# pinellolab/GRAFIMO

Hardware: AMD Instinct MI355X
Metric: scored haplotype k-mers/sec (higher is better)
Workload: dtype int32

## Files before the change

grafimo_amd/csrc/gfm_score_kernels.hpp:

```cpp
#pragma once

#include "gfm_common.hpp"

namespace {

constexpr int kWave = 64;
constexpr int kThreads = 1024;
constexpr int kWavesPerWG = kThreads / kWave;
constexpr unsigned kPoison = 0xFFFFu;
constexpr int kMaxLdsBytes = 160 * 1024;
constexpr int kWGsPerCU = 1;
constexpr int kReserveCUs = 4;
constexpr int kHitQueue = 64;

constexpr int kWorkspaces = GFM_WORKSPACE_RING;
constexpr int kCtlSlots = 2 * GFM_WORKSPACE_RING;
constexpr int kCtlAhead = GFM_WORKSPACE_RING;
struct HitCtl {
    unsigned long long mid[kCtlSlots];
    unsigned long long snap[kCtlSlots];
};
constexpr int kResidPerWG = kWavesPerWG * kHitQueue;

__device__ inline void hitq_push(long long *hitq, int &qn, bool hit, long long entry, int lane,
                                 const unsigned long long *hit_count, unsigned long long *mid,
                                 long long *hit_rows, long long hit_cap)
{
    const unsigned long long mask = __builtin_amdgcn_ballot_w64(hit);
    if (!mask) return;
    const int nh = __popcll(mask);
    if (qn + nh > kHitQueue) {
        unsigned long long base = 0;
        if (lane == 0) base = (hit_count ? *hit_count : 0ull) + atomicAdd(mid, (unsigned long long)qn);
        base = __shfl(base, 0);
        for (int i = lane; i < qn; i += kWave)
            if ((long long)(base + i) < hit_cap) hit_rows[base + i] = hitq[i];
        qn = 0;
    }
    if (hit) hitq[qn + __popcll(mask & ((1ull << lane) - 1ull))] = entry;
    qn += nh;
}

template <int WAVES>
__device__ inline void hitq_finish(const long long *hitq, int qn, int *wq_n ,
                                   int wave, int lane, int tid, long long *resid, int *resid_n)
{
    if (lane == 0) wq_n[wave] = qn;
    __syncthreads();
    int base = 0, tot = 0;
#pragma unroll
    for (int w = 0; w < WAVES; ++w) {
        if (w < wave) base += wq_n[w];
        tot += wq_n[w];
    }
    long long *slab = resid + (size_t)blockIdx.x * kResidPerWG;
    for (int i = lane; i < qn; i += kWave) slab[base + i] = hitq[i];
    if (tid == 0) resid_n[blockIdx.x] = tot;
}

constexpr int kSpillCopies = 16;

struct MotifArgs {
    const uint16_t *tab;
    int lo, nb, min_val;
    int use_hist;
    int spill_lo;
    int spill_n;
    unsigned *spill;
    int cutoff;
    int slot;
    int *scores;
    unsigned *partials;
    long long *hit_rows;
    long long hit_cap;
    const unsigned long long *hit_count;
    HitCtl *ctl;
    long long *resid;
    int *resid_n;
};
template <int MM> struct ScoreArgs {
    MotifArgs m[MM];
    int store_through;
};

typedef __attribute__((address_space(3))) const unsigned lds_cu32;
typedef __attribute__((address_space(3))) const uint16_t lds_cu16;
typedef __attribute__((address_space(3))) const unsigned long long lds_cu64;
__device__ inline unsigned lds_offset(const void *p)
{
    return (unsigned)(size_t)(__attribute__((address_space(3))) const char *)p;
}

constexpr int kSlabsPerGroup = 16;
constexpr int kPostJobs = 3;
struct PostJob {
    const unsigned *partials;
    unsigned long long *hist64;
    unsigned *spill;
    const long long *resid;
    const int *resid_n;
    HitCtl *ctl;
    long long *hit_rows;
    unsigned long long *hit_count;
    long long hit_cap;
    int nslabs, nb, lo, min_val, bin_blocks, hist_blocks, spill_lo, spill_n, spill_blocks, hit_slabs, par, total;
};
struct PostJobs { PostJob j[kPostJobs]; };

__device__ inline void
post_body(const unsigned *__restrict__ partials, int nslabs, int nb, int lo, int min_val,
          unsigned long long *__restrict__ hist64, int bin_blocks, int hist_blocks,
          unsigned *__restrict__ spill, int spill_lo, int spill_n, int spill_blocks,
          const long long *__restrict__ resid, const int *__restrict__ resid_n, int hit_slabs,
          HitCtl *__restrict__ ctl, int par, long long *__restrict__ hit_rows, long long hit_cap,
          unsigned long long *__restrict__ hit_count)
{
    const int tid = threadIdx.x;
    if (blockIdx.x == 0 && tid == 0 && hit_slabs == 0 && ctl) ctl->mid[(par + kCtlAhead) % kCtlSlots] = 0ull;
    if ((int)blockIdx.x < hist_blocks) {
        const int bx = blockIdx.x % bin_blocks, by = blockIdx.x / bin_blocks;
        const int b = bx * 256 + tid;
        if (b > nb) return;
        const int g0 = by * kSlabsPerGroup;
        const int g1 = min(g0 + kSlabsPerGroup, nslabs);
        unsigned long long s = 0;
        const size_t stride = (size_t)(nb + 1);
#pragma unroll 8
        for (int g = g0; g < g1; ++g) s += __builtin_nontemporal_load(&partials[g * stride + b]);
        if (s) atomicAdd(&hist64[b == nb ? min_val : lo + b], s);
        return;
    }
    if ((int)blockIdx.x < hist_blocks + spill_blocks) {
        const int b = ((int)blockIdx.x - hist_blocks) * 256 + tid;
        if (b < spill_n) {
            unsigned long long v = 0;
#pragma unroll
            for (int c = 0; c < kSpillCopies; ++c) {
                const unsigned x = spill[(size_t)c * (size_t)spill_n + b];
                if (x) {
                    v += x;
                    spill[(size_t)c * (size_t)spill_n + b] = 0u;
                }
            }
            if (v) atomicAdd(&hist64[spill_lo + b], v);
        }
        return;
    }
    __shared__ int part[256];
    __shared__ int part_all[256];
    const int g = blockIdx.x - hist_blocks - spill_blocks;
    int s = 0, sa = 0;
    for (int k = tid; k < hit_slabs; k += 256) {
        const int v = resid_n[k];
        sa += v;
        if (k < g) s += v;
    }
    part[tid] = s;
    part_all[tid] = sa;
    __syncthreads();
    for (int d = 128; d > 0; d >>= 1) {
        if (tid < d) { part[tid] += part[tid + d]; part_all[tid] += part_all[tid + d]; }
        __syncthreads();
    }
    const unsigned long long start = ctl->snap[par] + ctl->mid[par];
    const unsigned long long base = start + (unsigned long long)part[0];
    const int cnt = resid_n[g];
    const long long *slab = resid + (size_t)g * kResidPerWG;
    for (int i = tid; i < cnt; i += 256)
        if ((long long)(base + i) < hit_cap) __builtin_nontemporal_store(__builtin_nontemporal_load(&slab[i]), &hit_rows[base + i]);
    if (g == 0 && tid == 0) {
        *hit_count = start + (unsigned long long)part_all[0];
        ctl->mid[(par + kCtlAhead) % kCtlSlots] = 0ull;
    }
}

__global__ void __launch_bounds__(256) post_kernel(const PostJobs jobs)
{
    const PostJob &q = jobs.j[blockIdx.y];
    if ((int)blockIdx.x >= q.total) return;
    post_body(q.partials, q.nslabs, q.nb, q.lo, q.min_val, q.hist64, q.bin_blocks, q.hist_blocks, q.spill, q.spill_lo,
              q.spill_n, q.spill_blocks, q.resid, q.resid_n, q.hit_slabs, q.ctl, q.par, q.hit_rows, q.hit_cap,
              q.hit_count);
}

constexpr int kSelThreads = 256;
__global__ void __launch_bounds__(kSelThreads)
select_hits_kernel(const int *__restrict__ scores, long long n, const int *__restrict__ cutoff_ptr,
                   long long row_base, long long *__restrict__ hit_rows, long long hit_cap,
                   const unsigned long long *__restrict__ hit_count, HitCtl *__restrict__ ctl,
                   int par, long long *__restrict__ resid, int *__restrict__ resid_n,
                   const unsigned long long *__restrict__ gate_count, long long gate_cap)
{
    __shared__ long long hq[kSelThreads / kWave][kHitQueue];
    __shared__ int wq_n[kSelThreads / kWave];
    const int cutoff = *cutoff_ptr;
    const int tid = threadIdx.x, lane = tid & 63, wave = tid >> 6;
    long long *hitq = hq[wave];
    int qn = 0;
    if (gate_count) {
        if ((long long)*gate_count <= gate_cap) {
            if (tid == 0) {
                resid_n[blockIdx.x] = 0;
                if (blockIdx.x == 0) ctl->snap[par] = hit_count ? *hit_count : 0ull;
            }
            return;
        }
        hit_count = nullptr;
    }
    if (blockIdx.x == 0 && tid == 0) ctl->snap[par] = hit_count ? *hit_count : 0ull;
    const long long nthreads = (long long)gridDim.x * blockDim.x;
    const long long n4 = (n + 3) >> 2;
    const long long iters = (n4 + nthreads - 1) / nthreads;
    const long long t0 = (long long)blockIdx.x * blockDim.x + tid;
    for (long long it = 0; it < iters; ++it) {
        const long long i = t0 + it * nthreads;
        int sc[4] = {INT32_MIN, INT32_MIN, INT32_MIN, INT32_MIN};
        if (i * 4 + 4 <= n) {
            const int4 v = reinterpret_cast<const int4 *>(scores)[i];
            sc[0] = v.x; sc[1] = v.y; sc[2] = v.z; sc[3] = v.w;
        } else {
            for (int j = 0; j < 4; ++j)
                if (i * 4 + j < n) sc[j] = scores[i * 4 + j];
        }
#pragma unroll
        for (int j = 0; j < 4; ++j)
            hitq_push(hitq, qn, sc[j] >= cutoff,
                      ((row_base + i * 4 + j) << GFM_HIT_SCORE_BITS) | (long long)sc[j], lane,
                      hit_count, &ctl->mid[par], hit_rows, hit_cap);
    }
    hitq_finish<kSelThreads / kWave>(hitq, qn, wq_n, wave, lane, tid, resid, resid_n);
}

constexpr int kFilterPerThread = 16;
constexpr int kFilterPerBlock = kSelThreads * kFilterPerThread;
__global__ void __launch_bounds__(kSelThreads)
filter_hits_kernel(const long long *__restrict__ cand, const unsigned long long *__restrict__ cand_count,
                   long long cand_cap, const int *__restrict__ cutoff_ptr, long long *__restrict__ hit_rows,
                   long long hit_cap, unsigned long long *__restrict__ hit_count)
{
    __shared__ int wave_tot[kSelThreads / kWave];
    __shared__ unsigned long long block_base;
    const int cutoff = *cutoff_ptr;
    const int tid = threadIdx.x, lane = tid & 63, wave = tid >> 6;
    const unsigned long long have = *cand_count;
    if ((long long)have > cand_cap) {
        if (blockIdx.x == 0 && tid == 0) *hit_count = have;
        return;
    }
    const long long n = (long long)have;
    const long long first = (long long)blockIdx.x * kFilterPerBlock;
    if (first >= n) return;
    long long e[kFilterPerThread];
    int mine = 0;
#pragma unroll
    for (int j = 0; j < kFilterPerThread; ++j) {
        const long long i = first + (long long)j * kSelThreads + tid;
        e[j] = i < n ? cand[i] : -1ll;
        const bool keep = i < n && (int)(e[j] & ((1ll << GFM_HIT_SCORE_BITS) - 1)) >= cutoff;
        if (!keep) e[j] = -1ll;
        mine += keep ? 1 : 0;
    }
    int incl = mine;
#pragma unroll
    for (int d = 1; d < kWave; d <<= 1) {
        const int v = __shfl_up(incl, d);
        if (lane >= d) incl += v;
    }
    if (lane == kWave - 1) wave_tot[wave] = incl;
    __syncthreads();
    int before = 0, total = 0;
#pragma unroll
    for (int w = 0; w < kSelThreads / kWave; ++w) {
        if (w < wave) before += wave_tot[w];
        total += wave_tot[w];
    }
    if (tid == 0) block_base = total ? atomicAdd(hit_count, (unsigned long long)total) : 0ull;
    __syncthreads();
    unsigned long long at = block_base + (unsigned long long)(before + incl - mine);
#pragma unroll
    for (int j = 0; j < kFilterPerThread; ++j)
        if (e[j] >= 0) {
            if ((long long)at < hit_cap) hit_rows[at] = e[j];
            ++at;
        }
}

}
```

grafimo_amd/csrc/gfm_score_quad.hpp:

```cpp
#pragma once

#include "gfm_score_kernels.hpp"
#include "gfm_quad_launch.hpp"

namespace {

typedef unsigned u32x2_t __attribute__((ext_vector_type(2)));
typedef unsigned u32x4_t __attribute__((ext_vector_type(4)));
typedef __attribute__((address_space(3))) const u32x2_t lds_cu32x2;
typedef __attribute__((address_space(3))) const u32x4_t lds_cu32x4;
typedef int i32x4 __attribute__((ext_vector_type(4)));

template <int W, int MM, bool STORE = true>
__global__ void __launch_bounds__(kThreads)
score_quad_kernel(const uint8_t *__restrict__ kmers, long long n, long long row_base, const ScoreArgs<MM> a)
{
    extern __shared__ __attribute__((aligned(16))) unsigned char smem[];
    constexpr int NDW = (W + 3) / 4;
    constexpr int kTabBytes = quad_tab_bytes(W, MM);
    constexpr int CB = kQuadRows * W;
    constexpr int kLoads = (CB + 1023) / 1024;
    constexpr int GP = quad_pitch(W);
    constexpr int PAD = quad_pad(W);
    constexpr int SSTRIDE = quad_strip_stride(W, MM);

    if (lds_offset(smem) != 0u) __builtin_trap();
    const int tid = threadIdx.x;
    const int lane = tid & (kWave - 1);
    const int wave = __builtin_amdgcn_readfirstlane(tid >> 6);
    const int n_waves = (int)(blockDim.x >> 6);
    const int wg_threads = (int)blockDim.x;
    unsigned char *tab = smem;
    unsigned char *stage_base = smem + kTabBytes;
    unsigned *hist[MM];
    {
        unsigned *h = reinterpret_cast<unsigned *>(stage_base + n_waves * SSTRIDE);
#pragma unroll
        for (int m = 0; m < MM; ++m) {
            hist[m] = h;
            if (a.m[m].use_hist) h += a.m[m].nb + 1;
        }
    }

    unsigned char *stage = stage_base + wave * SSTRIDE;
    const unsigned stage_off = (unsigned)(kTabBytes + wave * SSTRIDE);
    const long long nfull = n / kQuadRows;
    const long long cstride = (long long)gridDim.x * n_waves;
    bool vec_store = true;
    const bool through = a.store_through == 1;
    constexpr bool no_store = !STORE;
#pragma unroll
    for (int m = 0; m < MM; ++m) vec_store = vec_store && (reinterpret_cast<uintptr_t>(a.m[m].scores) & 15u) == 0;

    uint4 pre[kQuadDepth][kLoads];
    auto fetch = [&](uint4 (&dst)[kLoads], long long c) {
        const uint8_t *src = kmers + c * (long long)CB + lane * 16;
#pragma unroll
        for (int i = 0; i < kLoads; ++i) {
            if (i * 1024 + 1024 <= CB || i * 1024 + lane * 16 < CB) {
                typedef unsigned u32x4 __attribute__((ext_vector_type(4)));
                const u32x4 t = __builtin_nontemporal_load(reinterpret_cast<const u32x4 *>(src + i * 1024));
                dst[i] = make_uint4(t.x, t.y, t.z, t.w);
            }
        }
    };

    long long *hitq[MM];
    int qn[MM];
    bool select[MM];
#pragma unroll
    for (int m = 0; m < MM; ++m) {
        hitq[m] = reinterpret_cast<long long *>(stage + quad_stage_bytes(W)) + m * kHitQueue;
        qn[m] = 0;
        select[m] = a.m[m].cutoff != GFM_NO_SELECT;
        if (select[m] && blockIdx.x == 0 && tid == 0)
            a.m[m].ctl->snap[a.m[m].slot] = a.m[m].hit_count ? *a.m[m].hit_count : 0ull;
    }

    int p_score[MM][4];
    long long p_crow = -1;
    auto book = [&]() {
        const int k0 = 4 * lane;
#pragma unroll
        for (int m = 0; m < MM; ++m) {
            const MotifArgs &ma = a.m[m];
            if (ma.use_hist) {
#pragma unroll
                for (int j = 0; j < 4; ++j) {
                    const unsigned off = (unsigned)(p_score[m][j] - ma.lo);
                    if (off < (unsigned)ma.nb)
                        atomicAdd(&hist[m][off], 1u);
                    else if (p_score[m][j] == ma.min_val)
                        atomicAdd(&hist[m][ma.nb], 1u);
                    else
                        atomicAdd(&ma.spill[(size_t)(blockIdx.x & (kSpillCopies - 1)) * (size_t)ma.spill_n + (size_t)(p_score[m][j] - ma.spill_lo)], 1u);
                }
            }
            if (select[m]) {
                const int best = max(max(p_score[m][0], p_score[m][1]), max(p_score[m][2], p_score[m][3]));
                if (__builtin_amdgcn_ballot_w64(best >= ma.cutoff)) {
#pragma unroll
                    for (int j = 0; j < 4; ++j)
                        hitq_push(hitq[m], qn[m], p_score[m][j] >= ma.cutoff,
                                  ((row_base + p_crow + k0 + j) << GFM_HIT_SCORE_BITS) | (long long)p_score[m][j], lane,
                                  ma.hit_count, &ma.ctl->mid[ma.slot], ma.hit_rows, ma.hit_cap);
                }
            }
        }
    };

    long long c = (long long)blockIdx.x * n_waves + wave;
#pragma unroll
    for (int d = 0; d < kQuadDepth; ++d)
        if (c + d * cstride < nfull) fetch(pre[d], c + d * cstride);
    if constexpr (MM == 1) {
        for (int i = tid; i < kTabBytes / 2; i += wg_threads) reinterpret_cast<uint16_t *>(tab)[i] = a.m[0].tab[i];
    } else {
        for (int i = tid; i < kTabBytes / 8; i += wg_threads) {
            unsigned long long v = 0;
            if (a.m[0].tab[i] == kPoison) {
                v = 1ull << 57;
            } else {
#pragma unroll
                for (int m = 0; m < MM; ++m) v |= (unsigned long long)a.m[m].tab[i] << (19 * m);
            }
            reinterpret_cast<unsigned long long *>(tab)[i] = v;
        }
    }
#pragma unroll
    for (int m = 0; m < MM; ++m)
        if (a.m[m].use_hist)
            for (int i = tid; i <= a.m[m].nb; i += wg_threads) hist[m][i] = 0u;
    __syncthreads();

    while (c < nfull) {
#pragma unroll
        for (int d = 0; d < kQuadDepth; ++d) {
            if (c >= nfull) break;
            const long long crow = c * kQuadRows;
            if (p_crow >= 0) book();
#pragma unroll
            for (int i = 0; i < kLoads; ++i) {
                const int off = i * 1024 + lane * 16;
                if (i * 1024 + 1024 <= CB || off < CB) {
                    const int dst = PAD ? off + PAD * (off / (4 * W)) : off;
                    *reinterpret_cast<uint4 *>(stage + dst) = pre[d][i];
                }
            }
            if (c + kQuadDepth * cstride < nfull) fetch(pre[d], c + kQuadDepth * cstride);
            __builtin_amdgcn_fence(__ATOMIC_RELEASE, "wavefront");
            __builtin_amdgcn_wave_barrier();

            unsigned w[W + 1];
            {
                const unsigned base = stage_off + (unsigned)(lane * GP);
                if constexpr (W % 2 == 1) {
#pragma unroll
                    for (int t = 0; t < W; ++t) w[t] = ((lds_cu32 *)(uintptr_t)base)[t];
                } else if constexpr (W % 4 == 2) {
#pragma unroll
                    for (int t = 0; t < W / 2; ++t) {
                        const u32x2_t v = ((lds_cu32x2 *)(uintptr_t)base)[t];
                        w[2 * t] = v.x;
                        w[2 * t + 1] = v.y;
                    }
                } else {
#pragma unroll
                    for (int t = 0; t < W / 4; ++t) {
                        const u32x4_t v = ((lds_cu32x4 *)(uintptr_t)base)[t];
                        w[4 * t] = v.x;
                        w[4 * t + 1] = v.y;
                        w[4 * t + 2] = v.z;
                        w[4 * t + 3] = v.w;
                    }
                }
                w[W] = 0u;
            }
            int score[MM][4];
#pragma unroll
            for (int j = 0; j < 4; ++j) {
                const int r = (j * W) & 3;
                bool any_n;
                int acc[MM];
                if constexpr (MM == 1) {
                    int s1 = 0;
#pragma unroll
                    for (int t = 0; t < NDW; ++t) {
                        const int q = (j * W + 4 * t) >> 2;
                        const unsigned x = r ? __builtin_amdgcn_alignbit(w[q + 1], w[q], (unsigned)(8 * r)) : w[q];
                        unsigned y;
                        asm("v_bfi_b32 %0, %1, %2, %3" : "=v"(y) : "s"(0x000E000Eu), "v"(x), "v"(x >> 5));
                        const unsigned e0 = y & 0x7Eu;
                        const unsigned e1 = (y >> 16) & 0x7Eu;
                        s1 += *(lds_cu16 *)(uintptr_t)(e0 + (unsigned)((2 * t) * 128));
                        s1 += *(lds_cu16 *)(uintptr_t)(e1 + (unsigned)((2 * t + 1) * 128));
                    }
                    any_n = (unsigned)s1 >= kPoison;
                    acc[0] = s1;
                } else {
                    unsigned long long s64 = 0;
#pragma unroll
                    for (int t = 0; t < NDW; ++t) {
                        const int q = (j * W + 4 * t) >> 2;
                        const unsigned x = r ? __builtin_amdgcn_alignbit(w[q + 1], w[q], (unsigned)(8 * r)) : w[q];
                        unsigned y;
                        asm("v_bfi_b32 %0, %1, %2, %3" : "=v"(y) : "s"(0x000E000Eu), "v"(x), "v"(x >> 5));
                        const unsigned e0 = (y & 0x7Eu) << 2;
                        const unsigned e1 = ((y >> 16) & 0x7Eu) << 2;
                        s64 += *(lds_cu64 *)(uintptr_t)(e0 + (unsigned)((2 * t) * 512));
                        s64 += *(lds_cu64 *)(uintptr_t)(e1 + (unsigned)((2 * t + 1) * 512));
                    }
                    any_n = (s64 >> 57) != 0;
#pragma unroll
                    for (int m = 0; m < MM; ++m) acc[m] = (int)((s64 >> (19 * m)) & 0x7FFFFull);
                }
#pragma unroll
                for (int m = 0; m < MM; ++m) score[m][j] = any_n ? a.m[m].min_val : acc[m];
            }
            const int k0 = 4 * lane;
#pragma unroll
            for (int m = 0; m < MM; ++m) {
                const __amdgpu_buffer_rsrc_t rs =
                    __builtin_amdgcn_make_buffer_rsrc(a.m[m].scores + crow, 0, kQuadRows * 4, 0x00020000);
                if (no_store) {
                } else if (vec_store) {
                    const u32x4_t out = {(unsigned)score[m][0], (unsigned)score[m][1], (unsigned)score[m][2],
                                         (unsigned)score[m][3]};
                    if (through)
                        __builtin_amdgcn_raw_buffer_store_b128(out, rs, k0 * 4, 0, kStoreThrough);
                    else
                        __builtin_amdgcn_raw_buffer_store_b128(out, rs, k0 * 4, 0, kStoreStream);
                } else {
#pragma unroll
                    for (int j = 0; j < 4; ++j) {
                        if (through)
                            __builtin_amdgcn_raw_buffer_store_b32((unsigned)score[m][j], rs, (k0 + j) * 4, 0, kStoreThrough);
                        else
                            __builtin_amdgcn_raw_buffer_store_b32((unsigned)score[m][j], rs, (k0 + j) * 4, 0, kStoreStream);
                    }
                }
#pragma unroll
                for (int j = 0; j < 4; ++j) p_score[m][j] = score[m][j];
            }
            p_crow = crow;
            __builtin_amdgcn_fence(__ATOMIC_ACQUIRE, "wavefront");
            __builtin_amdgcn_wave_barrier();
            c += cstride;
        }
    }
    if (p_crow >= 0) book();
    if (blockIdx.x == gridDim.x - 1 && wave == n_waves - 1 && nfull * kQuadRows < n) {
        const long long first = nfull * kQuadRows;
        const int count = (int)(n - first);
#pragma unroll 1
        for (int r0 = 0; r0 < count; r0 += kWave) {
            const int k = r0 + lane;
            const bool live = k < count;
            const uint8_t *row = kmers + (first + (live ? k : 0)) * (long long)W;
            unsigned long long s64 = 0;
            bool bad = false;
#pragma unroll 1
            for (int p = 0; p < 2 * NDW; ++p) {
                const unsigned b0 = 2 * p < W ? row[2 * p] : (unsigned)'A';
                const unsigned b1 = 2 * p + 1 < W ? row[2 * p + 1] : (unsigned)'A';
                const unsigned e = p * 64 + ((b0 >> 1) & 7u) + 8u * ((b1 >> 1) & 7u);
                if constexpr (MM == 1) {
                    const unsigned v = reinterpret_cast<const uint16_t *>(tab)[e];
                    bad = bad || v == kPoison;
                    s64 += v;
                } else {
                    s64 += reinterpret_cast<const unsigned long long *>(tab)[e];
                }
            }
            if constexpr (MM > 1) bad = (s64 >> 57) != 0;
#pragma unroll
            for (int m = 0; m < MM; ++m) {
                const MotifArgs &ma = a.m[m];
                const int sc = bad ? ma.min_val : (int)((MM == 1 ? s64 : (s64 >> (19 * m))) & 0x7FFFFull);
                if (live) {
                    if (!no_store) ma.scores[first + k] = sc;
                    if (ma.use_hist) {
                        const unsigned off = (unsigned)(sc - ma.lo);
                        if (off < (unsigned)ma.nb)
                            atomicAdd(&hist[m][off], 1u);
                        else if (sc == ma.min_val)
                            atomicAdd(&hist[m][ma.nb], 1u);
                        else
                            atomicAdd(&ma.spill[(size_t)(blockIdx.x & (kSpillCopies - 1)) * (size_t)ma.spill_n + (size_t)(sc - ma.spill_lo)], 1u);
                    }
                }
                if (select[m])
                    hitq_push(hitq[m], qn[m], live && sc >= ma.cutoff,
                              ((row_base + first + k) << GFM_HIT_SCORE_BITS) | (long long)sc, lane, ma.hit_count,
                              &ma.ctl->mid[ma.slot], ma.hit_rows, ma.hit_cap);
            }
        }
    }

    __syncthreads();
#pragma unroll
    for (int m = 0; m < MM; ++m) {
        const MotifArgs &ma = a.m[m];
        if (select[m]) {
            int *wq_n = reinterpret_cast<int *>(tab) + m * kWavesPerWG;
            if (lane == 0) wq_n[wave] = qn[m];
            __syncthreads();
            int base = 0, tot = 0;
            for (int w2 = 0; w2 < n_waves; ++w2) {
                const int v = wq_n[w2];
                if (w2 < wave) base += v;
                tot += v;
            }
            long long *slab = ma.resid + (size_t)blockIdx.x * kResidPerWG;
            for (int i = lane; i < qn[m]; i += kWave) slab[base + i] = hitq[m][i];
            if (tid == 0) ma.resid_n[blockIdx.x] = tot;
        }
        if (ma.use_hist) {
            unsigned *slab = ma.partials + (size_t)blockIdx.x * (size_t)(ma.nb + 1);
            for (int i = tid; i <= ma.nb; i += wg_threads) slab[i] = hist[m][i];
        }
    }
}

}
```

Baseline: 218.4 billion.

## Defer score stores to next iteration and use explicit LDS atomics for histogram

Score stores now happen one iteration late, issued after the next chunk is staged into LDS, so global writes overlap with the following fetch and compute instead of sitting right after scoring. Histogram updates go through a helper that does workgroup-scoped relaxed LDS atomic adds at a precomputed LDS byte offset, and the two in-window branches are merged into one. The cost is keeping previous scores live longer, which may raise register pressure. The no_store check inside the main loop appears to be replaced by the STORE template parameter.

```diff
diff --git a/grafimo_amd/csrc/gfm_score_kernels.hpp b/grafimo_amd/csrc/gfm_score_kernels.hpp
--- a/grafimo_amd/csrc/gfm_score_kernels.hpp
+++ b/grafimo_amd/csrc/gfm_score_kernels.hpp
@@ -86,9 +86,14 @@
 typedef __attribute__((address_space(3))) const unsigned lds_cu32;
 typedef __attribute__((address_space(3))) const uint16_t lds_cu16;
 typedef __attribute__((address_space(3))) const unsigned long long lds_cu64;
+typedef __attribute__((address_space(3))) unsigned lds_u32;
 __device__ inline unsigned lds_offset(const void *p)
 {
     return (unsigned)(size_t)(__attribute__((address_space(3))) const char *)p;
+}
+__device__ inline void lds_count(unsigned byte_off, unsigned bin)
+{
+    __hip_atomic_fetch_add((lds_u32 *)(uintptr_t)byte_off + bin, 1u, __ATOMIC_RELAXED, __HIP_MEMORY_SCOPE_WORKGROUP);
 }
 
 constexpr int kSlabsPerGroup = 16;
diff --git a/grafimo_amd/csrc/gfm_score_quad.hpp b/grafimo_amd/csrc/gfm_score_quad.hpp
--- a/grafimo_amd/csrc/gfm_score_quad.hpp
+++ b/grafimo_amd/csrc/gfm_score_quad.hpp
@@ -77,6 +77,17 @@
             a.m[m].ctl->snap[a.m[m].slot] = a.m[m].hit_count ? *a.m[m].hit_count : 0ull;
     }
 
+    unsigned hist_off[MM];
+#pragma unroll
+    for (int m = 0; m < MM; ++m) hist_off[m] = lds_offset(hist[m]);
+    auto count_row = [&](const MotifArgs &ma, unsigned h_off, int sc) {
+        const unsigned off = (unsigned)(sc - ma.lo);
+        const bool in_win = off < (unsigned)ma.nb;
+        if (in_win || sc == ma.min_val)
+            lds_count(h_off, in_win ? off : (unsigned)ma.nb);
+        else
+            atomicAdd(&ma.spill[(size_t)(blockIdx.x & (kSpillCopies - 1)) * (size_t)ma.spill_n + (size_t)(sc - ma.spill_lo)], 1u);
+    };
     int p_score[MM][4];
     long long p_crow = -1;
     auto book = [&]() {
@@ -86,15 +97,7 @@
             const MotifArgs &ma = a.m[m];
             if (ma.use_hist) {
 #pragma unroll
-                for (int j = 0; j < 4; ++j) {
-                    const unsigned off = (unsigned)(p_score[m][j] - ma.lo);
-                    if (off < (unsigned)ma.nb)
-                        atomicAdd(&hist[m][off], 1u);
-                    else if (p_score[m][j] == ma.min_val)
-                        atomicAdd(&hist[m][ma.nb], 1u);
-                    else
-                        atomicAdd(&ma.spill[(size_t)(blockIdx.x & (kSpillCopies - 1)) * (size_t)ma.spill_n + (size_t)(p_score[m][j] - ma.spill_lo)], 1u);
-                }
+                for (int j = 0; j < 4; ++j) count_row(ma, hist_off[m], p_score[m][j]);
             }
             if (select[m]) {
                 const int best = max(max(p_score[m][0], p_score[m][1]), max(p_score[m][2], p_score[m][3]));
@@ -104,6 +107,32 @@
                         hitq_push(hitq[m], qn[m], p_score[m][j] >= ma.cutoff,
                                   ((row_base + p_crow + k0 + j) << GFM_HIT_SCORE_BITS) | (long long)p_score[m][j], lane,
                                   ma.hit_count, &ma.ctl->mid[ma.slot], ma.hit_rows, ma.hit_cap);
+                }
+            }
+        }
+    };
+    auto store_prev = [&]() {
+        if constexpr (STORE) {
+            const int k0 = 4 * lane;
+#pragma unroll
+            for (int m = 0; m < MM; ++m) {
+                const __amdgpu_buffer_rsrc_t rs =
+                    __builtin_amdgcn_make_buffer_rsrc(a.m[m].scores + p_crow, 0, kQuadRows * 4, 0x00020000);
+                if (vec_store) {
+                    const u32x4_t out = {(unsigned)p_score[m][0], (unsigned)p_score[m][1], (unsigned)p_score[m][2],
+                                         (unsigned)p_score[m][3]};
+                    if (through)
+                        __builtin_amdgcn_raw_buffer_store_b128(out, rs, k0 * 4, 0, kStoreThrough);
+                    else
+                        __builtin_amdgcn_raw_buffer_store_b128(out, rs, k0 * 4, 0, kStoreStream);
+                } else {
+#pragma unroll
+                    for (int j = 0; j < 4; ++j) {
+                        if (through)
+                            __builtin_amdgcn_raw_buffer_store_b32((unsigned)p_score[m][j], rs, (k0 + j) * 4, 0, kStoreThrough);
+                        else
+                            __builtin_amdgcn_raw_buffer_store_b32((unsigned)p_score[m][j], rs, (k0 + j) * 4, 0, kStoreStream);
+                    }
                 }
             }
         }
@@ -147,6 +176,7 @@
                     *reinterpret_cast<uint4 *>(stage + dst) = pre[d][i];
                 }
             }
+            if (p_crow >= 0) store_prev();
             if (c + kQuadDepth * cstride < nfull) fetch(pre[d], c + kQuadDepth * cstride);
             __builtin_amdgcn_fence(__ATOMIC_RELEASE, "wavefront");
             __builtin_amdgcn_wave_barrier();
@@ -217,28 +247,8 @@
 #pragma unroll
                 for (int m = 0; m < MM; ++m) score[m][j] = any_n ? a.m[m].min_val : acc[m];
             }
-            const int k0 = 4 * lane;
 #pragma unroll
             for (int m = 0; m < MM; ++m) {
-                const __amdgpu_buffer_rsrc_t rs =
-                    __builtin_amdgcn_make_buffer_rsrc(a.m[m].scores + crow, 0, kQuadRows * 4, 0x00020000);
-                if (no_store) {
-                } else if (vec_store) {
-                    const u32x4_t out = {(unsigned)score[m][0], (unsigned)score[m][1], (unsigned)score[m][2],
-                                         (unsigned)score[m][3]};
-                    if (through)
-                        __builtin_amdgcn_raw_buffer_store_b128(out, rs, k0 * 4, 0, kStoreThrough);
-                    else
-                        __builtin_amdgcn_raw_buffer_store_b128(out, rs, k0 * 4, 0, kStoreStream);
-                } else {
-#pragma unroll
-                    for (int j = 0; j < 4; ++j) {
-                        if (through)
-                            __builtin_amdgcn_raw_buffer_store_b32((unsigned)score[m][j], rs, (k0 + j) * 4, 0, kStoreThrough);
-                        else
-                            __builtin_amdgcn_raw_buffer_store_b32((unsigned)score[m][j], rs, (k0 + j) * 4, 0, kStoreStream);
-                    }
-                }
 #pragma unroll
                 for (int j = 0; j < 4; ++j) p_score[m][j] = score[m][j];
             }
@@ -248,7 +258,10 @@
             c += cstride;
         }
     }
-    if (p_crow >= 0) book();
+    if (p_crow >= 0) {
+        store_prev();
+        book();
+    }
     if (blockIdx.x == gridDim.x - 1 && wave == n_waves - 1 && nfull * kQuadRows < n) {
         const long long first = nfull * kQuadRows;
         const int count = (int)(n - first);
@@ -279,15 +292,7 @@
                 const int sc = bad ? ma.min_val : (int)((MM == 1 ? s64 : (s64 >> (19 * m))) & 0x7FFFFull);
                 if (live) {
                     if (!no_store) ma.scores[first + k] = sc;
-                    if (ma.use_hist) {
-                        const unsigned off = (unsigned)(sc - ma.lo);
-                        if (off < (unsigned)ma.nb)
-                            atomicAdd(&hist[m][off], 1u);
-                        else if (sc == ma.min_val)
-                            atomicAdd(&hist[m][ma.nb], 1u);
-                        else
-                            atomicAdd(&ma.spill[(size_t)(blockIdx.x & (kSpillCopies - 1)) * (size_t)ma.spill_n + (size_t)(sc - ma.spill_lo)], 1u);
-                    }
+                    if (ma.use_hist) count_row(ma, hist_off[m], sc);
                 }
                 if (select[m])
                     hitq_push(hitq[m], qn[m], live && sc >= ma.cutoff,
```

Measured after the change: 208.6 billion. 0.955x the previous value.
